# google-research/se3ds

Hardware: AMD Instinct MI355X
Metric: panoramas/sec (G+D train step) at 512x1024 RGB-D (higher is better)
Workload: dtype bf16; 1 GPU; configs/highres 512x1024 full GAN step train_g_d (G+D+hinge+depth+wc losses, clip, Adam, EMA), ResNet-101 gen_dims 128, per-GPU batch 8, d_step_per_g_step 1; per_gpu_batch=8, global_batch=8, parallelism=dp1

## Files before the change

### include/se3ds_hip.h

```cpp
#ifndef SE3DS_HIP_H_
#define SE3DS_HIP_H_

#include <stddef.h>
#include <stdint.h>

#ifdef __cplusplus
extern "C" {
#endif

#define SE3DS_OK 0
#define SE3DS_E_BADSHAPE (-1)
#define SE3DS_E_BADDTYPE (-2)
#define SE3DS_E_WORKSPACE (-3)
#define SE3DS_E_LAUNCH (-4)
#define SE3DS_E_UNSUPPORTED (-5)

#define SE3DS_F32 0
#define SE3DS_I32 1
#define SE3DS_U8 2
#define SE3DS_BF16 3
#define SE3DS_FEAT_BYTE_RANGE 0x100
#define SE3DS_XYZ1_ONES_PRESET 0x200

const char* se3ds_version(void);
// ... 249 lines not shown
int se3ds_pad2d(const void* x, int dtype, int n, int h, int w, int c, int pad, int mode, int wrap_w,
                float value, void* y, void* stream);
int se3ds_head_fwd(const void* x, int dtype, int64_t n, int kind, float* y, void* stream);
int se3ds_head_bwd(const float* dy, const float* y, const void* x, int dtype, int64_t n, int kind,
                   void* dx, void* stream);

int se3ds_sample_sum(const float* a, const float* b, const float* m, int n, int64_t p, int c,
                     int mode, float* out, float* workspace , void* stream);
int se3ds_l1_grad(const float* a, const float* b, const float* m, const float* m2,
                  const float* coef, int n, int64_t p, int c, int mode, float* grad, void* stream);
int se3ds_recip_clamp(const float* sums, int n, float scale, float* out, void* stream);
int se3ds_hinge(const void* logits, int dtype, int64_t half, float cd, float cg, float* sums,
                void* dlog_d, void* dlog_g, void* stream);

int se3ds_multi_sqnorm(const float* grads, const int64_t* chunks, int64_t nchunks,
                       const int64_t* tensor_chunk_start, int ntensors, float* partial,
                       float* sqnorm, void* stream);
int se3ds_multi_clip_by_norm(float* grads, const int64_t* chunks, int64_t nchunks,
                             const float* sqnorm, int ntensors, float clip_norm,
                             float* mean_norm_out, void* stream);
int se3ds_mean_clipped_norm(const float* sqnorm, int ntensors, float clip_norm, float* out,
                            void* stream);
int se3ds_multi_adam_keras(float* params, const float* grads, float* m, float* v, int64_t n,
                           float lr, float beta1, float beta2, float eps, int64_t step,
                           void* stream);
int se3ds_multi_adam_keras_ema(float* params, const float* grads, float* m, float* v, int64_t n,
                               float lr, float beta1, float beta2, float eps, int64_t step,
                               float* ema, float one_minus_decay, void* stream);
int se3ds_multi_clip_adam_keras_ema(float* params, const float* grads, float* m, float* v,
                                    const int64_t* chunks, int64_t nchunks, const float* sqnorm,
                                    float clip_norm, const int64_t* tensor_sn, float lr, float beta1,
                                    float beta2, float eps, int64_t step, float* ema,
                                    float one_minus_decay, void* stream);
int se3ds_multi_ema(float* ema, const float* vars, int64_t n, float one_minus_decay, void* stream);

int se3ds_spectral_table_fields(void);
int se3ds_spectral_part_rows(void);
int se3ds_spectral_vpart_len(void);
int se3ds_spectral_power_iter(const int64_t* table, int nlayers, int training, void* stream);
int se3ds_spectral_bwd_fixup(const int64_t* table, int nlayers, void* stream);
int se3ds_spectral_bwd_dots(const int64_t* table, int nlayers, void* stream);
int se3ds_multi_sqnorm_sn(const float* grads, const int64_t* chunks, int64_t nchunks,
                          const int64_t* tensor_chunk_start, int ntensors, float* partial,
                          float* sqnorm, const int64_t* tensor_sn, int tensor_base, void* stream);
int se3ds_multi_clip_by_norm_sn(float* grads, const int64_t* chunks, int64_t nchunks,
                                const float* sqnorm, int ntensors, float clip_norm,
                                float* mean_norm_out, const int64_t* tensor_sn, void* stream);


int se3ds_input_transform(const uint8_t* image, const uint8_t* proj_image, const uint16_t* depth,
                          const uint16_t* proj_depth, const uint8_t* proj_mask,
                          const uint8_t* blurred_mask, const uint8_t* segmentation,
                          const int32_t* iparams, const float* fparams, int n, int h0, int w0, int h,
                          int w, float* o_image, float* o_proj_image, float* o_proj_mask,
                          float* o_proj_depth, float* o_depth, float* o_blurred, int32_t* o_seg,
                          void* stream);

int se3ds_video_transform(const float* image, const uint8_t* segmentation,
                          const uint8_t* pd_segmentation, const float* depth, const float* pd_depth,
                          const int32_t* hmode, const float* hband, int n, int t, int h0, int w0,
                          int h, int w, float* o_original, float* o_image, uint8_t* o_seg,
                          uint8_t* o_pd_seg, float* o_depth, float* o_pd_depth, void* stream);

int se3ds_png_unfilter(const uint8_t* src, int64_t src_bytes, const int64_t* table,
                       const int64_t* host_table, int n, void* stream);
int se3ds_png_unfilter_fields(void);
int se3ds_png_unfilter_max_row_bytes(void);

int se3ds_png_inflate(const uint8_t* buf, int64_t buf_bytes, uint8_t* workspace,
                      int64_t workspace_bytes, const int64_t* host_table, int n,
                      int32_t* status_dev, void* stream);
int se3ds_png_inflate_fields(void);
int se3ds_png_inflate_ring_bytes(void);

// ... 31 lines not shown
```

### se3ds_amd/csrc/optim.hip

```cpp
#include "common.h"
#include <cmath>

namespace se3ds {
namespace {

constexpr int kB = 256;

__global__ void __launch_bounds__(kB)
chunk_sqsum_kernel(const float* __restrict__ g, const int64_t* __restrict__ chunks,
                   float* __restrict__ partial, const int64_t* __restrict__ tensor_sn) {
  __shared__ float sh[kB / 64];
  const int64_t start = chunks[blockIdx.x * 3 + 1], len = chunks[blockIdx.x * 3 + 2];
  if (tensor_sn && tensor_sn[chunks[blockIdx.x * 3]] != 0) {
    if (threadIdx.x == 0) partial[blockIdx.x] = 0.f;
    return;
  }
  float s = 0.f;
  const float* gp = g + start;
  const int64_t n4 = (((uintptr_t)gp & 15) == 0) ? (len >> 2) : 0;
  float s1 = 0.f, s2 = 0.f, s3 = 0.f;
  for (int64_t i = threadIdx.x; i < n4; i += kB) {
    const float4 v = reinterpret_cast<const float4*>(gp)[i];
    s += v.x * v.x;
    s1 += v.y * v.y;
// ... 187 lines not shown
      const int c = (int)(e - k * C);
      const float vk = sv[k];
      const float4 u4 = *reinterpret_cast<const float4*>(su + c);
      gc[0] = clip_sn(g4.x, inv, coef, vk, u4.x, clip, den);
      gc[1] = clip_sn(g4.y, inv, coef, vk, u4.y, clip, den);
      gc[2] = clip_sn(g4.z, inv, coef, vk, u4.z, clip, den);
      gc[3] = clip_sn(g4.w, inv, coef, vk, u4.w, clip, den);
    }
    adam_elem(gc[0], p4.x, m4.x, v4.x, alpha, b1, b2, eps);
    adam_elem(gc[1], p4.y, m4.y, v4.y, alpha, b1, b2, eps);
    adam_elem(gc[2], p4.z, m4.z, v4.z, alpha, b1, b2, eps);
    adam_elem(gc[3], p4.w, m4.w, v4.w, alpha, b1, b2, eps);
    *reinterpret_cast<float4*>(m + o) = m4;
    *reinterpret_cast<float4*>(v + o) = v4;
    *reinterpret_cast<float4*>(p + o) = p4;
    if (EMA) {
      float4 e4 = *reinterpret_cast<const float4*>(ema + o);
      e4.x = ema_elem(e4.x, p4.x, omd); e4.y = ema_elem(e4.y, p4.y, omd);
      e4.z = ema_elem(e4.z, p4.z, omd); e4.w = ema_elem(e4.w, p4.w, omd);
      *reinterpret_cast<float4*>(ema + o) = e4;
    }
  }
  for (int64_t i = len4 + threadIdx.x; i < len; i += kB) {
    const int64_t o = start + i;
    float pi = p[o], mi = m[o], vi = v[o];
    adam_elem(one(i, g[o]), pi, mi, vi, alpha, b1, b2, eps);
    m[o] = mi;
    v[o] = vi;
    p[o] = pi;
    if (EMA) ema[o] = ema_elem(ema[o], pi, omd);
  }
}

__global__ void __launch_bounds__(kB)
ema_kernel(float* __restrict__ ema, const float* __restrict__ var, int64_t n, float omd) {
  for (int64_t i = (int64_t)blockIdx.x * kB + threadIdx.x; i < n; i += (int64_t)gridDim.x * kB)
    ema[i] = ema[i] - (ema[i] - var[i]) * omd;
}

constexpr int SN_F = 10;
constexpr int SN_KB = 32;
constexpr float SN_EPS = 1e-10f;

__global__ void __launch_bounds__(kB)
sn_v_kernel(const int64_t* __restrict__ tab) {
  const int64_t* L = tab + (int64_t)blockIdx.y * SN_F;
  const float* W = (const float*)L[0];
  const float* u = (const float*)L[1];
  float* v = (float*)L[2];
  float* vpart = (float*)L[6];
  const int64_t K = L[7];
  const int C = (int)L[8];
  __shared__ float sh[kB / 64];
  const int lane = threadIdx.x & 63, wave = threadIdx.x >> 6;
  float sq = 0.f;
  for (int64_t k = (int64_t)blockIdx.x * 4 + wave; k < K; k += (int64_t)SN_RB * 4) {
    float s = 0.f;
    for (int c = lane; c < C; c += 64) s += W[k * C + c] * u[c];
    s = wave_sum(s);
    if (lane == 0) { v[k] = s; sq += s * s; }
  }
  if (lane == 0) sh[wave] = sq;
  __syncthreads();
  if (threadIdx.x == 0) vpart[blockIdx.x] = (sh[0] + sh[1]) + (sh[2] + sh[3]);
}

// ... 139 lines not shown
        const float gv = G[k * C + c];
        dot += gv * W[k * C + c];
        gg += gv * gv;
        row += gv * uhat[c];
      }
    }
    gvu += row * vk;
  }
  dot = wave_sum(dot);
  gg = wave_sum(gg);
  gvu = wave_sum(gvu);
  if (lane == 0) { sh[0][wave] = dot; sh[1][wave] = gg; sh[2][wave] = gvu; }
  __syncthreads();
  if (threadIdx.x < 3) {
    const float* q = sh[threadIdx.x];
    vpart[threadIdx.x * SN_RB + blockIdx.x] = (q[0] + q[1]) + (q[2] + q[3]);
  }
  if (blockIdx.x == 0) {
    __syncthreads();
    float nv = 0.f, nu = 0.f;
    for (int64_t k = threadIdx.x; k < K; k += kB) nv += v[k] * v[k];
    for (int c = threadIdx.x; c < C; c += kB) nu += uhat[c] * uhat[c];
    nv = wave_sum(nv);
    nu = wave_sum(nu);
    if (lane == 0) { sh[0][wave] = nv; sh[1][wave] = nu; }
    __syncthreads();
    if (threadIdx.x < 2) {
      const float* q = sh[threadIdx.x];
      vpart[3 * SN_RB + threadIdx.x] = (q[0] + q[1]) + (q[2] + q[3]);
    }
  }
}

__global__ void __launch_bounds__(kB)
sn_sqnorm_kernel(const int64_t* __restrict__ tensor_sn, int tensor_base, int T,
                 float* __restrict__ sqnorm) {
  for (int t = blockIdx.x * kB + threadIdx.x; t < T; t += gridDim.x * kB) {
    const int64_t* L = (const int64_t*)tensor_sn[tensor_base + t];
    if (L == nullptr) continue;
    const float* sig = (const float*)L[4];
    const float* vpart = (const float*)L[6];
    const float dot = sn_dot_gw(vpart);
    double gg = 0.0, gvu = 0.0;
    for (int i = 0; i < SN_RB; ++i) {
      gg += (double)vpart[SN_RB + i];
      gvu += (double)vpart[2 * SN_RB + i];
    }
    const float inv = sig[1];
    const float coef = inv * inv * dot;
    const double nvu = (double)vpart[3 * SN_RB] * (double)vpart[3 * SN_RB + 1];
    double sq = (double)inv * inv * gg - 2.0 * (double)inv * coef * gvu + (double)coef * coef * nvu;
    sqnorm[t] = sq > 0.0 ? (float)sq : 0.f;
  }
}

}
}

using namespace se3ds;

static float adam_alpha(float lr, float beta1, float beta2, int64_t step) {
  float b1p = (float)pow((double)beta1, (double)step);
  float b2p = (float)pow((double)beta2, (double)step);
  return lr * sqrtf(1.0f - b2p) / (1.0f - b1p);
}

// ... 62 lines not shown

int se3ds_multi_adam_keras_ema(float* params, const float* grads, float* m, float* v, int64_t n,
                               float lr, float beta1, float beta2, float eps, int64_t step,
                               float* ema, float one_minus_decay, void* stream) {
  if (ema == nullptr)
    return se3ds_multi_adam_keras(params, grads, m, v, n, lr, beta1, beta2, eps, step, stream);
  if (n <= 0) return SE3DS_OK;
  float alpha = adam_alpha(lr, beta1, beta2, step);
  hipLaunchKernelGGL(adam_ema_kernel, dim3(grid_for(n, kB)), dim3(kB), 0, as_stream(stream), params,
                     grads, m, v, n, alpha, beta1, beta2, eps, ema, one_minus_decay);
  return check_launch("multi_adam_keras_ema");
}

int se3ds_multi_clip_adam_keras_ema(float* params, const float* grads, float* m, float* v,
                                    const int64_t* chunks, int64_t nchunks, const float* sqnorm,
                                    float clip_norm, const int64_t* tensor_sn, float lr, float beta1,
                                    float beta2, float eps, int64_t step, float* ema,
                                    float one_minus_decay, void* stream) {
  if (nchunks <= 0) return SE3DS_OK;
  if ((((uintptr_t)params | (uintptr_t)grads | (uintptr_t)m | (uintptr_t)v | (uintptr_t)ema) & 15) != 0)
    return SE3DS_E_UNSUPPORTED;
  const float alpha = adam_alpha(lr, beta1, beta2, step);
  if (ema)
    hipLaunchKernelGGL(clip_adam_kernel<true>, dim3((unsigned)nchunks), dim3(kB), 0, as_stream(stream),
                       params, grads, m, v, chunks, sqnorm, clip_norm, tensor_sn, alpha, beta1, beta2,
                       eps, ema, one_minus_decay);
  else
    hipLaunchKernelGGL(clip_adam_kernel<false>, dim3((unsigned)nchunks), dim3(kB), 0, as_stream(stream),
                       params, grads, m, v, chunks, sqnorm, clip_norm, tensor_sn, alpha, beta1, beta2,
                       eps, ema, one_minus_decay);
  return check_launch("multi_clip_adam_keras_ema");
}

int se3ds_multi_ema(float* ema, const float* vars, int64_t n, float one_minus_decay,
                    void* stream) {
  if (n <= 0) return SE3DS_OK;
  hipLaunchKernelGGL(ema_kernel, dim3(grid_for(n, kB)), dim3(kB), 0, as_stream(stream), ema, vars,
                     n, one_minus_decay);
  return check_launch("multi_ema");
}

int se3ds_spectral_power_iter(const int64_t* table, int nlayers, int training, void* stream) {
  if (nlayers <= 0) return SE3DS_OK;
  hipStream_t s = as_stream(stream);
  hipLaunchKernelGGL(sn_v_kernel, dim3(SN_RB, (unsigned)nlayers), dim3(kB), 0, s, table);
  hipLaunchKernelGGL(sn_u_kernel, dim3(SN_KB, (unsigned)nlayers), dim3(kB), 0, s, table);
  hipLaunchKernelGGL(sn_finish_kernel, dim3((unsigned)nlayers), dim3(kB), 0, s, table, training);
  return check_launch("spectral_power_iter");
}

int se3ds_spectral_bwd_fixup(const int64_t* table, int nlayers, void* stream) {
  if (nlayers <= 0) return SE3DS_OK;
  hipStream_t s = as_stream(stream);
  hipLaunchKernelGGL(sn_dot_kernel, dim3(SN_RB, (unsigned)nlayers), dim3(kB), 0, s, table);
  hipLaunchKernelGGL(sn_fix_kernel, dim3(SN_RB, (unsigned)nlayers), dim3(kB), 0, s, table);
  return check_launch("spectral_bwd_fixup");
}

int se3ds_spectral_bwd_dots(const int64_t* table, int nlayers, void* stream) {
  if (nlayers <= 0) return SE3DS_OK;
  hipLaunchKernelGGL(sn_dots_kernel, dim3(SN_RB, (unsigned)nlayers), dim3(kB), 0, as_stream(stream),
                     table);
  return check_launch("spectral_bwd_dots");
}

int se3ds_spectral_table_fields(void) { return SN_F; }
int se3ds_spectral_part_rows(void) { return SN_KB; }
int se3ds_spectral_vpart_len(void) { return 3 * SN_RB + 2; }

}
```

### se3ds_amd/hipops/__init__.py

```python
import ctypes

from se3ds_amd import _lib
from se3ds_amd._lib import c_int, c_i64, c_f, c_p, c_sz

_lib.register({
    'se3ds_weight_prep': (c_int, [c_p, c_i64, c_int, c_int, c_p, c_p, c_p]),
    'se3ds_weight_prep_multi': (c_int, [c_p, c_int, c_i64, c_p]),
    'se3ds_conv2d_fwd': (c_int, [c_p, c_p, c_p, c_int] + [c_int] * 13 + [c_p, c_int, c_p, c_p, c_p,
                                                                      c_p, c_int, c_f, c_p]),
    'se3ds_conv2d_fwd_stats': (c_int, [c_p, c_p, c_p, c_int] + [c_int] * 13 + [c_p, c_int, c_p, c_p,
                                                                            c_p, c_p, c_int, c_f, c_p,
                                                                            c_p]),
    'se3ds_conv2d_fwd_stats_rows': (c_i64, [c_int] * 11),
    'se3ds_conv_transpose2x2_fwd': (c_int, [c_p, c_p, c_p, c_int, c_int, c_int, c_int, c_int, c_int, c_p, c_p]),
    'se3ds_conv2d_dgrad': (c_int, [c_p, c_p, c_p, c_int] + [c_int] * 13 + [c_p, c_p, c_p, c_p,
                                                                        c_int, c_f, c_p]),
    'se3ds_conv2d_dgrad_acc': (c_int, [c_p, c_p, c_p, c_int] + [c_int] * 13 + [c_p, c_p, c_p, c_p,
                                                                        c_int, c_f, c_p, c_p]),
    'se3ds_conv2d_dgrad_bnstats_rows': (c_i64, [c_int] * 10),
    'se3ds_conv2d_dgrad_bnstats': (c_int, [c_p, c_p, c_p, c_int] + [c_int] * 13 +
                                   [c_p, c_p, c_p, c_p, c_p, c_p, c_p, c_int, c_f, c_p, c_p]),
    'se3ds_conv2d_wgrad_workspace_bytes': (c_sz, [c_int] * 7),
    'se3ds_conv2d_wgrad': (c_int, [c_p, c_p, c_p, c_int] + [c_int] * 13 + [c_p, c_int, c_p, c_p, c_int,
                                                                        c_p, c_sz, c_p]),
# ... 28 lines not shown
    'se3ds_norm_bwd_cg_col_rows': (c_int, [c_i64, c_int]),
    'se3ds_norm_bwd_cg': (c_int, [c_p, c_p, c_int, c_i64, c_int, c_p, c_p, c_p, c_f, c_int, c_f, c_p,
                                  c_p, c_p, c_int, c_f, c_p, c_p, c_p, c_p, c_p, c_p, c_p, c_sz, c_p]),
    'se3ds_norm_bwd_apply_rows': (c_int, [c_p, c_p, c_int, c_i64, c_int, c_p, c_p, c_p, c_p, c_f,
                                          c_int, c_f, c_p, c_p, c_p, c_p, c_p, c_p, c_p, c_sz, c_p]),
    'se3ds_affine_bwd': (c_int, [c_p, c_p, c_int, c_int, c_i64, c_int, c_p, c_int, c_f, c_p, c_p,
                                 c_p, c_p]),
    'se3ds_act_bwd': (c_int, [c_p, c_p, c_int, c_i64, c_int, c_f, c_p, c_p]),
    'se3ds_add': (c_int, [c_p, c_p, c_int, c_i64, c_p, c_p]),
    'se3ds_row_scale': (c_int, [c_p, c_int, c_i64, c_int, c_p, c_p, c_p]),
    'se3ds_maxpool2x2_fwd': (c_int, [c_p, c_int, c_int, c_int, c_int, c_int, c_p, c_p]),
    'se3ds_maxpool2x2_bwd': (c_int, [c_p, c_p, c_p, c_int, c_int, c_int, c_int, c_int, c_p, c_p]),
    'se3ds_avgpool3s2_fwd': (c_int, [c_p, c_int, c_int, c_int, c_int, c_int, c_p, c_p]),
    'se3ds_avgpool3s2_bwd': (c_int, [c_p, c_int, c_int, c_int, c_int, c_int, c_p, c_p]),
    'se3ds_upsample2x_fwd': (c_int, [c_p, c_int, c_int, c_int, c_int, c_int, c_p, c_p]),
    'se3ds_upsample2x_bwd': (c_int, [c_p, c_int, c_int, c_int, c_int, c_int, c_p, c_p]),
    'se3ds_copy_channels': (c_int, [c_p, c_int, c_int, c_int, c_p, c_int, c_int, c_int, c_int,
                                    c_i64, c_p]),
    'se3ds_fill': (c_int, [c_p, c_int, c_i64, c_f, c_p]),
    'se3ds_head_fwd': (c_int, [c_p, c_int, c_i64, c_int, c_p, c_p]),
    'se3ds_head_bwd': (c_int, [c_p, c_p, c_p, c_int, c_i64, c_int, c_p, c_p]),
    'se3ds_sample_sum': (c_int, [c_p, c_p, c_p, c_int, c_i64, c_int, c_int, c_p, c_p, c_p]),
    'se3ds_l1_grad': (c_int, [c_p, c_p, c_p, c_p, c_p, c_int, c_i64, c_int, c_int, c_p, c_p]),
    'se3ds_recip_clamp': (c_int, [c_p, c_int, c_f, c_p, c_p]),
    'se3ds_hinge': (c_int, [c_p, c_int, c_i64, c_f, c_f, c_p, c_p, c_p, c_p]),
    'se3ds_multi_sqnorm': (c_int, [c_p, c_p, c_i64, c_p, c_int, c_p, c_p, c_p]),
    'se3ds_multi_clip_by_norm': (c_int, [c_p, c_p, c_i64, c_p, c_int, c_f, c_p, c_p]),
    'se3ds_mean_clipped_norm': (c_int, [c_p, c_int, c_f, c_p, c_p]),
    'se3ds_multi_adam_keras': (c_int, [c_p, c_p, c_p, c_p, c_i64, c_f, c_f, c_f, c_f, c_i64, c_p]),
    'se3ds_multi_adam_keras_ema': (c_int, [c_p, c_p, c_p, c_p, c_i64, c_f, c_f, c_f, c_f, c_i64, c_p,
                                           c_f, c_p]),
    'se3ds_multi_clip_adam_keras_ema': (c_int, [c_p, c_p, c_p, c_p, c_p, c_i64, c_p, c_f, c_p, c_f, c_f,
                                                c_f, c_f, c_i64, c_p, c_f, c_p]),
    'se3ds_multi_ema': (c_int, [c_p, c_p, c_i64, c_f, c_p]),
    'se3ds_spectral_table_fields': (c_int, []),
    'se3ds_spectral_part_rows': (c_int, []),
    'se3ds_spectral_vpart_len': (c_int, []),
    'se3ds_spectral_power_iter': (c_int, [c_p, c_int, c_int, c_p]),
    'se3ds_spectral_bwd_fixup': (c_int, [c_p, c_int, c_p]),
    'se3ds_spectral_bwd_dots': (c_int, [c_p, c_int, c_p]),
    'se3ds_multi_sqnorm_sn': (c_int, [c_p, c_p, c_i64, c_p, c_int, c_p, c_p, c_p, c_int, c_p]),
    'se3ds_multi_clip_by_norm_sn': (c_int, [c_p, c_p, c_i64, c_p, c_int, c_f, c_p, c_p, c_p]),
    'se3ds_quantize': (c_int, [c_p, c_int, c_i64, c_int, c_f, c_f, c_f, c_f, c_f, c_f, c_p, c_int, c_p]),
    'se3ds_pad2d': (c_int, [c_p, c_int, c_int, c_int, c_int, c_int, c_int, c_int, c_int, c_f, c_p,
                            c_p]),
})
```

### se3ds_amd/hipops/nn.py

```python
import math
import threading
from typing import List, Optional

import numpy as np
import os

import torch
import torch.distributed as dist

from se3ds_amd import _lib
from se3ds_amd import hipops

ACT_NONE, ACT_RELU, ACT_LRELU = 0, 1, 2
BN_EPS, BN_MOMENTUM = 1e-3, 0.99
IN_EPS = 1e-3


def _L():
  return _lib.lib()


def _log_collective(kind, numel):
  from se3ds_amd.trainers import dist_utils
  dist_utils.log_collective(kind, numel)


def _all_reduce_sum(t, group, kind):
  from se3ds_amd.trainers import dist_utils
  dist_utils.all_reduce_sum(t, group, kind)


def _chk(rc, what):
# ... 664 lines not shown
    self._copies[dtype] = (version, wt, wn)
    return wt, wn


class OperandGroup:

  def __init__(self, layers: List['ConvLayer'], dtype, device):
    self.dtype = dtype
    self.batched, self.single, rows, tile0 = [], [], [], 0
    for l in layers:
      w = l.kernel
      K, co = w.shape[0] * w.shape[1] * w.shape[2], w.shape[3]
      if dtype == torch.bfloat16 and K % 8 == 0 and co % 4 == 0:
        ent = l._copies.get(dtype)
        if ent is None:
          wt = torch.empty((co, K), dtype=dtype, device=w.device)
          wn = torch.empty((K, co), dtype=dtype, device=w.device)
          l._copies[dtype] = (-1, wt, wn)
        else:
          wt, wn = ent[1], ent[2]
        if (w.data_ptr() | wt.data_ptr()) % 16 == 0 and wn.data_ptr() % 8 == 0:
          rows.append([w.data_ptr(), K, co, wt.data_ptr(), wn.data_ptr(), tile0])
          tile0 += ((K + 63) // 64) * ((co + 63) // 64)
          self.batched.append(l)
          continue
      self.single.append(l)
    self.tiles = tile0
    self.table = torch.tensor(rows, dtype=torch.int64, device=device) if rows else None

  def prep(self, version):
    if self.table is not None:
      _chk(_L().se3ds_weight_prep_multi(self.table.data_ptr(), len(self.batched), self.tiles,
                                        _lib.stream()), 'se3ds_weight_prep_multi')
      for l in self.batched:
        ent = l._copies[self.dtype]
        l._copies[self.dtype] = (version, ent[1], ent[2])
    for l in self.single:
      l.prep(self.dtype, version)


class SpectralGroup:

  def __init__(self, layers: List[ConvLayer], device):
    self.layers = [l for l in layers if l.spectral]
    L = _L()
    nf, pr, vl = (L.se3ds_spectral_table_fields(), L.se3ds_spectral_part_rows(),
                  L.se3ds_spectral_vpart_len())
    rows = []
    for l in self.layers:
      w = l.kernel
      K, co = w.shape[0] * w.shape[1] * w.shape[2], w.shape[3]
      l.sn = dict(v=torch.zeros(K, device=device), uhat=torch.zeros(co, device=device),
                  sig=torch.ones(2, device=device), part=torch.zeros(pr * co, device=device),
                  vpart=torch.zeros(vl, device=device))
      rows.append([w.data_ptr(), l.store[l.name + '/u'].data_ptr(), l.sn['v'].data_ptr(),
                   l.sn['uhat'].data_ptr(), l.sn['sig'].data_ptr(), l.sn['part'].data_ptr(),
                   l.sn['vpart'].data_ptr(), K, co, 0])
      assert len(rows[-1]) == nf
    self._rows = rows
    self.table = torch.tensor(rows, dtype=torch.int64, device=device) if rows else None
    self._eff = [i for i, l in enumerate(self.layers) if l.kind == 'spectral']
    self._eff_table = None

  @property
  def eff_table(self):
    if self._eff_table is None and self._eff:
      rows = []
      for i in self._eff:
        l = self.layers[i]
        r = list(self._rows[i])
        r[9] = l.store.grad_views[l.name + '/kernel'].data_ptr()
        rows.append(r)
      self._eff_table = torch.tensor(rows, dtype=torch.int64, device=self.table.device)
    return self._eff_table

  def power_iteration(self, training):
    if self.table is not None:
      _chk(_L().se3ds_spectral_power_iter(self.table.data_ptr(), self.table.shape[0],
                                          1 if training else 0, _lib.stream()),
           'se3ds_spectral_power_iter')

  def tensor_sn(self, store):
    tab = self.eff_table
    if tab is None:
      return None
    if getattr(self, '_tensor_sn', None) is None:
      nf = tab.shape[1]
      index = {n_: t for t, n_ in enumerate(store.trainable_names)}
      rows = [0] * len(store.trainable_names)
      for j, i in enumerate(self._eff):
        rows[index[self.layers[i].name + '/kernel']] = tab.data_ptr() + 8 * nf * j
      self._tensor_sn = torch.tensor(rows, dtype=torch.int64, device=tab.device)
    return self._tensor_sn

  def backward_fixup(self, prefix=None, dots_only=False):
    tab = self.eff_table
    if tab is None:
      return
    if prefix is not None:
      cache = self.__dict__.setdefault('_seg_tables', {})
      if prefix not in cache:
        pres = prefix if isinstance(prefix, (tuple, list)) else (prefix,)
        rows = [j for j, i in enumerate(self._eff)
                if any(self.layers[i].name.startswith(pre + '/') for pre in pres)]
        cache[prefix] = tab[rows].contiguous() if rows else None
      tab = cache[prefix]
      if tab is None:
        return
    if dots_only:
      _chk(_L().se3ds_spectral_bwd_dots(tab.data_ptr(), tab.shape[0], _lib.stream()),
           'se3ds_spectral_bwd_dots')
      return
    _chk(_L().se3ds_spectral_bwd_fixup(tab.data_ptr(), tab.shape[0], _lib.stream()),
         'se3ds_spectral_bwd_fixup')


_CHECK_MASKS = os.environ.get('SE3DS_CHECK_MASKS') == '1'


def mask_window(ctx, mask, n, h, w, ho, wo, k, stride, pad_t, pad_l, wrap, want_bwd):
  if _CHECK_MASKS and ctx.binary_masks and not bool(((mask == 0) | (mask == 1)).all()):
    raise _lib.Se3dsHipError('a partial-conv mask with values outside {0, 1} reached a binary-mask fast path: '
                             'set gan.binary_masks = False (ctx.binary_masks) for fractional masks')
  ratio = torch.empty((n, ho, wo), dtype=torch.float32, device=ctx.device)
  um = torch.empty_like(ratio)
  ru = torch.empty_like(ratio) if want_bwd else None
  bu = torch.empty_like(ratio) if want_bwd else None
  _chk(_L().se3ds_mask_window(mask.data_ptr(), n, h, w, ho, wo, k, k, stride, pad_t, pad_l,
                              1 if wrap else 0, ratio.data_ptr(), um.data_ptr(), _lib.ptr(ru),
                              _lib.ptr(bu), _lib.stream()), 'se3ds_mask_window')
  return ratio, um, ru, bu


def _colsum(ctx, t2d_ptr, dtype_code, rows, c, row_scale=None, groups=1, out=None):
  sums = torch.empty((groups, 2, c), dtype=torch.float32, device=ctx.device)
  L = _L()
  ws = ctx.ws('norm', L.se3ds_norm_workspace_bytes(groups, c))
  _chk(L.se3ds_norm_stats(t2d_ptr, dtype_code, groups, rows, c, _lib.ptr(row_scale),
                          sums.data_ptr(), _lib.ptr(out), ws.data_ptr(), ws.numel(),
                          _lib.stream()), 'se3ds_norm_stats')
  return sums


_RED_TABLES = {}


def _wgrad(ctx, layer, args, wsz):
# ... 661 lines not shown
```

### se3ds_amd/trainers/gan_manager.py

```python
import abc
import csv
import os
import random
import re
import struct
import zlib
from typing import Optional

import numpy as np
import torch
import torch.distributed as dist

from se3ds_amd import _lib
from se3ds_amd import gin_lite as gin
from se3ds_amd import hipops
from se3ds_amd.trainers import dist_utils
from se3ds_amd.utils import ema


class OneDeviceStrategy:
  num_replicas_in_sync = 1
  group = None

  def __init__(self, device='cuda:0'):
    self.device = torch.device(device)


class DataParallelStrategy:

  def __init__(self, device, group=None):
    self.device = torch.device(device)
    self.group = group
    self.num_replicas_in_sync = dist.get_world_size(group)


class AdamState:

  def __init__(self, model, lr, beta_1, beta_2, epsilon=1e-7):
    self.model = model
    self.lr, self.beta_1, self.beta_2, self.epsilon = lr, beta_1, beta_2, epsilon
    self.m = torch.zeros_like(model.store.theta)
    self.v = torch.zeros_like(model.store.theta)
    self.iterations = 0
    self.chunks, self.tensor_chunk_start = model.store.chunk_tables()
    self._tcs_host = self.tensor_chunk_start.cpu().tolist()
    dev = model.store.theta.device
    self.partial = torch.empty(self.chunks.shape[0], dtype=torch.float32, device=dev)
    self.sqnorm = torch.empty(len(model.store.trainable_names), dtype=torch.float32, device=dev)
# ... 34 lines not shown
    tcs = cache[(t0, t1)]
    _lib.check(L.se3ds_multi_sqnorm_sn(st.grad.data_ptr(), self.chunks.data_ptr() + 24 * c0, c1 - c0,
                                       tcs.data_ptr(), t1 - t0, self.partial.data_ptr(),
                                       self.sqnorm.data_ptr() + 4 * t0, sn, t0, _lib.stream()),
               'se3ds_multi_sqnorm_sn')
    _lib.check(L.se3ds_multi_clip_by_norm_sn(st.grad.data_ptr(), self.chunks.data_ptr() + 24 * c0,
                                             c1 - c0, self.sqnorm.data_ptr(), t1 - t0,
                                             float(clip_norm), None, sn, _lib.stream()),
               'se3ds_multi_clip_by_norm_sn')

  def clip_apply(self, t0, t1, clip_norm=5.0, fused_sn=False, ema_theta=None, one_minus_decay=0.0):
    if self.on_update is not None:
      return False
    st = self.model.store
    L = _lib.lib()
    sn = self._sn_ptr(fused_sn)
    c0, c1 = self._tcs_host[t0], self._tcs_host[t1]
    if c1 <= c0:
      return True
    cache = self.__dict__.setdefault('_seg_tcs', {})
    if (t0, t1) not in cache:
      cache[(t0, t1)] = (self.tensor_chunk_start[t0:t1 + 1] - c0).contiguous()
    tcs = cache[(t0, t1)]
    _lib.check(L.se3ds_multi_sqnorm_sn(st.grad.data_ptr(), self.chunks.data_ptr() + 24 * c0, c1 - c0,
                                       tcs.data_ptr(), t1 - t0, self.partial.data_ptr(),
                                       self.sqnorm.data_ptr() + 4 * t0, sn, t0, _lib.stream()),
               'se3ds_multi_sqnorm_sn')
    _lib.check(L.se3ds_multi_clip_adam_keras_ema(
        st.theta.data_ptr(), st.grad.data_ptr(), self.m.data_ptr(), self.v.data_ptr(),
        self.chunks.data_ptr() + 24 * c0, c1 - c0, self.sqnorm.data_ptr(), float(clip_norm), sn,
        self.lr, self.beta_1, self.beta_2, self.epsilon, self.iterations, _lib.ptr(ema_theta),
        float(one_minus_decay), _lib.stream()), 'se3ds_multi_clip_adam_keras_ema')
    return True

  def mean_clipped_norm(self, clip_norm=5.0):
    _lib.check(_lib.lib().se3ds_mean_clipped_norm(
        self.sqnorm.data_ptr(), len(self.model.store.trainable_names), float(clip_norm),
        self.mean_norm.data_ptr(), _lib.stream()), 'se3ds_mean_clipped_norm')
    return self.mean_norm

  def begin_step(self):
    self.iterations += 1

  def apply_segment(self, e0, e1, ema_theta=None, one_minus_decay=0.0):
    st = self.model.store
    if e1 <= e0:
      return
    if self.on_update is not None:
      self.on_update(e0, e1)
    _lib.check(_lib.lib().se3ds_multi_adam_keras_ema(
        st.theta.data_ptr() + 4 * e0, st.grad.data_ptr() + 4 * e0, self.m.data_ptr() + 4 * e0,
        self.v.data_ptr() + 4 * e0, e1 - e0, self.lr, self.beta_1, self.beta_2, self.epsilon,
        self.iterations, (ema_theta.data_ptr() + 4 * e0) if ema_theta is not None else None,
        float(one_minus_decay), _lib.stream()), 'se3ds_multi_adam_keras_ema')

  def end_step(self):
    self.model.store.version += 1

  def apply_gradients(self, group=None, world=1, ema_theta=None, one_minus_decay=0.0):
    st = self.model.store
    if world > 1:
      dist_utils.allreduce_arena_sum(st.grad, group)
    if self.on_update is not None:
      self.on_update(0, st.theta.numel())
    self.iterations += 1
    _lib.check(_lib.lib().se3ds_multi_adam_keras_ema(
# ... 361 lines not shown
```

### se3ds_amd/trainers/se3ds_trainer.py

```python
import os
from typing import Dict

import torch

from se3ds_amd import _lib
from se3ds_amd import gin_lite as gin
from se3ds_amd.hipops import nn
from se3ds_amd.hipops.nn import Var
from se3ds_amd.models import image_models
from se3ds_amd.trainers import dist_utils
from se3ds_amd.trainers import gan_manager
from se3ds_amd.trainers.gan_manager import Mean

FUSED_SN_CLIP = True
GRAD_CLIP_NORM = 5.0
SEGMENT_OPTIMIZER = os.environ.get('SE3DS_SEGMENT_OPTIMIZER', '1') != '0'
FUSED_CLIP_ADAM = os.environ.get('SE3DS_FUSED_CLIP_ADAM', '1') != '0'
DEFER_WGRAD_REDUCE = os.environ.get('SE3DS_DEFER_WGRAD_REDUCE', '1') != '0'


def _L():
  return _lib.lib()


@gin.configurable(denylist=['strategy', 'model_dir'])
class GAN(gan_manager.GANManager):

  def __init__(self, lambda_gan, lambda_kld, lambda_wc, lambda_depth, *args,
               dis_use_pred_depth=True, mask_blurred=False, **kwargs):
    super().__init__(*args, **kwargs)
    self.lambda_gan = lambda_gan
    self.lambda_kld = lambda_kld
    self.lambda_wc = lambda_wc
    self.lambda_depth = lambda_depth
    self.dis_use_pred_depth = dis_use_pred_depth
    self.mask_blurred = mask_blurred

  def _create_metrics(self):
    names = ['gen/gen_loss', 'dis/disc_loss', 'dis/grad_norm', 'gen/gen_feat_loss',
             'gen/gen_gan_loss', 'gen/depth_loss', 'gen/seg_loss', 'gen/depth_seg_loss',
             'gen/depth_seg_consistency', 'gen/kld_loss', 'gen/kld_nan', 'gen/wc_loss',
             'gen/grad_norm']
    self.metrics = {n: Mean(n.split('/')[-1]) for n in names}

  def _prep_inputs(self, inputs):
    inputs = dict(inputs)
    for k in ('image', 'proj_image', 'proj_depth', 'proj_mask', 'depth', 'blurred_mask'):
      t = inputs[k]
      _lib.require_cuda(t)
      inputs[k] = t.to(torch.float32).contiguous()
    if not self.mask_blurred:
# ... 186 lines not shown
    gx = x_all.grad
    x_all.grad = None
    del tape_d
    g_rgb = nn.slice_channels(gx[:n], 0, 3, torch.float32)
    _lib.check(L.se3ds_add(d_rgb.data_ptr(), g_rgb.data_ptr(), _lib.F32, d_rgb.numel(),
                           d_rgb.data_ptr(), _lib.stream()), 'se3ds_add')
    if self.dis_use_pred_depth:
      g_dep = nn.slice_channels(gx[:n], 3, 1, torch.float32)
      _lib.check(L.se3ds_add(d_depth.data_ptr(), g_dep.data_ptr(), _lib.F32, d_depth.numel(),
                             d_depth.data_ptr(), _lib.stream()), 'se3ds_add')
    ctx_g.param_grads = True
    push_rgb(d_rgb)
    push_depth(d_depth)
    ema_theta, ema_omd = self.ema_fused_args()
    if sync is None and SEGMENT_OPTIMIZER and nn.conv_profiler() is None:
      segs = self._segments()
      opt = self._optimizer_stream(dev)
      main = torch.cuda.current_stream(dev)
      ev = torch.cuda.Event()
      ev.record()
      with torch.cuda.stream(opt):
        opt.wait_event(ev)
        self._update_all(self.d_optimizer, False, None, 0.0)
        d_norm = self.d_optimizer.mean_clipped_norm(GRAD_CLIP_NORM).clone()
      self.g_optimizer.begin_step()
      def segment_done(name):
        if name not in segs:
          return
        t0, t1, e0, e1 = segs[name]
        done = torch.cuda.Event()
        done.record()
        with torch.cuda.stream(opt):
          opt.wait_event(done)
          nn.flush_wgrad_reduces(ctx_g)
          G.spectral.backward_fixup(prefix=G.SEGMENTS[name], dots_only=FUSED_SN_CLIP)
          if not (FUSED_CLIP_ADAM and self.g_optimizer.clip_apply(
              t0, t1, GRAD_CLIP_NORM, FUSED_SN_CLIP, ema_theta, ema_omd)):
            self.g_optimizer.clip_segment(t0, t1, GRAD_CLIP_NORM, fused_sn=FUSED_SN_CLIP)
            self.g_optimizer.apply_segment(e0, e1, ema_theta, ema_omd)
          self._operand_group(G, name, ctx_g.dtype).prep(G.store.version + 1)
      ctx_g.on_segment = segment_done
      if DEFER_WGRAD_REDUCE:
        ctx_g.wgrad_defer = []
      ctx_g.backward()
      ctx_g.on_segment = None
      ctx_g.wgrad_defer = None
      with torch.cuda.stream(opt):
        opt.wait_stream(main)
        self._operand_group(D, None, ctx_d.dtype).prep(D.store.version)
      main.wait_stream(opt)
      self.g_optimizer.end_step()
      g_norm = self.g_optimizer.mean_clipped_norm(GRAD_CLIP_NORM).clone()
    elif sync is None:
      if DEFER_WGRAD_REDUCE:
        ctx_g.wgrad_defer = []
      ctx_g.backward()
      ctx_g.wgrad_defer = None
      G.spectral.backward_fixup(dots_only=FUSED_SN_CLIP)
      self._update_all(self.g_optimizer, FUSED_SN_CLIP, ema_theta, ema_omd)
      g_norm = self.g_optimizer.mean_clipped_norm(GRAD_CLIP_NORM).clone()
      self._update_all(self.d_optimizer, False, None, 0.0)
      d_norm = self.d_optimizer.mean_clipped_norm(GRAD_CLIP_NORM).clone()
      self._operand_group(G, None, ctx_g.dtype).prep(G.store.version)
      self._operand_group(D, None, ctx_d.dtype).prep(D.store.version)
    else:
      opt = self._optimizer_stream(dev)
      main = torch.cuda.current_stream(dev)
      opt.wait_stream(main)
      def segment_done(name):
        if name not in self._g_segments:
          return
        t0, t1, e0, e1 = self._g_segments[name]
        done = torch.cuda.Event()
# ... 91 lines not shown
```

Baseline: 42.45 panoramas/sec.

## Fuse clip+Adam+EMA with bf16 weight prep per generator segment

```diff
diff --git a/include/se3ds_hip.h b/include/se3ds_hip.h
--- a/include/se3ds_hip.h
+++ b/include/se3ds_hip.h
@@ -305,6 +305,11 @@
                                     float clip_norm, const int64_t* tensor_sn, float lr, float beta1,
                                     float beta2, float eps, int64_t step, float* ema,
                                     float one_minus_decay, void* stream);
+int se3ds_multi_clip_adam_keras_ema_prep(const int64_t* table, int nlayers, int64_t total_tiles,
+                                         const float* sqnorm, float clip_norm, float lr, float beta1,
+                                         float beta2, float eps, int64_t step, float one_minus_decay,
+                                         void* stream);
+int se3ds_clip_adam_prep_table_fields(void);
 int se3ds_multi_ema(float* ema, const float* vars, int64_t n, float one_minus_decay, void* stream);
 
 int se3ds_spectral_table_fields(void);
@@ -313,6 +318,8 @@
 int se3ds_spectral_power_iter(const int64_t* table, int nlayers, int training, void* stream);
 int se3ds_spectral_bwd_fixup(const int64_t* table, int nlayers, void* stream);
 int se3ds_spectral_bwd_dots(const int64_t* table, int nlayers, void* stream);
+int se3ds_spectral_bwd_dots_reduce(const int64_t* table, int nlayers, const int64_t* src_table,
+                                   void* stream);
 int se3ds_multi_sqnorm_sn(const float* grads, const int64_t* chunks, int64_t nchunks,
                           const int64_t* tensor_chunk_start, int ntensors, float* partial,
                           float* sqnorm, const int64_t* tensor_sn, int tensor_base, void* stream);
diff --git a/se3ds_amd/csrc/optim.hip b/se3ds_amd/csrc/optim.hip
--- a/se3ds_amd/csrc/optim.hip
+++ b/se3ds_amd/csrc/optim.hip
@@ -243,6 +243,111 @@
   }
 }
 
+constexpr int AP_F = 12;
+__global__ void __launch_bounds__(kB)
+clip_adam_prep_kernel(const int64_t* __restrict__ table, int nlayers, const float* __restrict__ sqnorm,
+                      float clip, float alpha, float b1, float b2, float eps, float omd) {
+  __shared__ float tile[64][65];
+  const int64_t blk = blockIdx.x;
+  int lo = 0, hi = nlayers - 1;
+  while (lo < hi) {
+    const int mid = (lo + hi + 1) >> 1;
+    if (table[(int64_t)mid * AP_F + 11] <= blk) lo = mid; else hi = mid - 1;
+  }
+  const int64_t* R = table + (int64_t)lo * AP_F;
+  float* __restrict__ p = (float*)R[0];
+  const float* __restrict__ g = (const float*)R[1];
+  float* __restrict__ m = (float*)R[2];
+  float* __restrict__ v = (float*)R[3];
+  float* __restrict__ ema = (float*)R[4];
+  uint16_t* __restrict__ wt = (uint16_t*)R[5];
+  uint16_t* __restrict__ wn = (uint16_t*)R[6];
+  const int64_t K = R[7];
+  const int Cout = (int)R[8];
+  const float sq = sqnorm[R[9]];
+  const float norm = sq > 0.f ? sqrtf(sq) : sq;
+  const float den = fmaxf(norm, clip);
+  const int64_t* L = (const int64_t*)R[10];
+  const float* sv = nullptr;
+  const float* su = nullptr;
+  float inv = 0.f, coef = 0.f;
+  if (L != nullptr) {
+    sv = (const float*)L[2];
+    su = (const float*)L[3];
+    const float* sig = (const float*)L[4];
+    const float* vpart = (const float*)L[6];
+    const float dot = sn_dot_gw(vpart);
+    inv = sig[1];
+    coef = inv * inv * dot;
+  }
+  const int64_t local = blk - R[11];
+  const int64_t tiles_k = (K + 63) / 64;
+  const int64_t k0 = (local % tiles_k) * 64;
+  const int c0 = (int)(local / tiles_k) * 64;
+  const int tid = threadIdx.x;
+  {
+    const int cq = (tid & 15) * 4, r0 = tid >> 4;
+#pragma unroll
+    for (int i = 0; i < 4; ++i) {
+      const int r = r0 + 16 * i;
+      const int64_t k = k0 + r;
+      const int c = c0 + cq;
+      float4 p4 = make_float4(0.f, 0.f, 0.f, 0.f);
+      if (k < K && c < Cout) {
+        const int64_t o = k * Cout + c;
+        const float4 g4 = *reinterpret_cast<const float4*>(g + o);
+        p4 = *reinterpret_cast<const float4*>(p + o);
+        float4 m4 = *reinterpret_cast<const float4*>(m + o);
+        float4 v4 = *reinterpret_cast<const float4*>(v + o);
+        float gc[4];
+        if (L == nullptr) {
+          gc[0] = clip_plain(g4.x, clip, den); gc[1] = clip_plain(g4.y, clip, den);
+          gc[2] = clip_plain(g4.z, clip, den); gc[3] = clip_plain(g4.w, clip, den);
+        } else {
+          const float vk = sv[k];
+          const float4 u4 = *reinterpret_cast<const float4*>(su + c);
+          gc[0] = clip_sn(g4.x, inv, coef, vk, u4.x, clip, den);
+          gc[1] = clip_sn(g4.y, inv, coef, vk, u4.y, clip, den);
+          gc[2] = clip_sn(g4.z, inv, coef, vk, u4.z, clip, den);
+          gc[3] = clip_sn(g4.w, inv, coef, vk, u4.w, clip, den);
+        }
+        adam_elem(gc[0], p4.x, m4.x, v4.x, alpha, b1, b2, eps);
+        adam_elem(gc[1], p4.y, m4.y, v4.y, alpha, b1, b2, eps);
+        adam_elem(gc[2], p4.z, m4.z, v4.z, alpha, b1, b2, eps);
+        adam_elem(gc[3], p4.w, m4.w, v4.w, alpha, b1, b2, eps);
+        *reinterpret_cast<float4*>(m + o) = m4;
+        *reinterpret_cast<float4*>(v + o) = v4;
+        *reinterpret_cast<float4*>(p + o) = p4;
+        if (ema != nullptr) {
+          float4 e4 = *reinterpret_cast<const float4*>(ema + o);
+          e4.x = ema_elem(e4.x, p4.x, omd); e4.y = ema_elem(e4.y, p4.y, omd);
+          e4.z = ema_elem(e4.z, p4.z, omd); e4.w = ema_elem(e4.w, p4.w, omd);
+          *reinterpret_cast<float4*>(ema + o) = e4;
+        }
+        uint16_t ob[4] = {f32_to_bf16(p4.x), f32_to_bf16(p4.y), f32_to_bf16(p4.z), f32_to_bf16(p4.w)};
+        *reinterpret_cast<uint2*>(wn + o) = *reinterpret_cast<const uint2*>(ob);
+      }
+      tile[r][cq] = p4.x; tile[r][cq + 1] = p4.y; tile[r][cq + 2] = p4.z; tile[r][cq + 3] = p4.w;
+    }
+  }
+  __syncthreads();
+  {
+    const int kq = (tid & 7) * 8, cr0 = tid >> 3;
+#pragma unroll
+    for (int j = 0; j < 2; ++j) {
+      const int cr = cr0 + 32 * j;
+      const int c = c0 + cr;
+      const int64_t k = k0 + kq;
+      if (c < Cout && k < K) {
+        uint16_t ob[8];
+#pragma unroll
+        for (int e = 0; e < 8; ++e) ob[e] = f32_to_bf16(tile[kq + e][cr]);
+        *reinterpret_cast<uint4*>(wt + (int64_t)c * K + k) = *reinterpret_cast<const uint4*>(ob);
+      }
+    }
+  }
+}
+
 __global__ void __launch_bounds__(kB)
 ema_kernel(float* __restrict__ ema, const float* __restrict__ var, int64_t n, float omd) {
   for (int64_t i = (int64_t)blockIdx.x * kB + threadIdx.x; i < n; i += (int64_t)gridDim.x * kB)
@@ -448,6 +553,111 @@
   }
 }
 
+__device__ __forceinline__ float4 slab_sum4(const float4* __restrict__ P, int splits, int64_t n4,
+                                            int64_t i) {
+  float4 s0 = make_float4(0.f, 0.f, 0.f, 0.f), s1 = s0, s2 = s0, s3 = s0;
+  auto add = [](float4& a, const float4& b) { a.x += b.x; a.y += b.y; a.z += b.z; a.w += b.w; };
+  int k = 0;
+  for (; k + 3 < splits; k += 4) {
+    const float4 a = P[(int64_t)k * n4 + i], b = P[(int64_t)(k + 1) * n4 + i];
+    const float4 c = P[(int64_t)(k + 2) * n4 + i], d = P[(int64_t)(k + 3) * n4 + i];
+    add(s0, a); add(s1, b); add(s2, c); add(s3, d);
+  }
+  for (; k < splits; ++k) add(s0, P[(int64_t)k * n4 + i]);
+  return make_float4(((s0.x + s1.x) + (s2.x + s3.x)) * 1.0f, ((s0.y + s1.y) + (s2.y + s3.y)) * 1.0f,
+                     ((s0.z + s1.z) + (s2.z + s3.z)) * 1.0f, ((s0.w + s1.w) + (s2.w + s3.w)) * 1.0f);
+}
+
+__global__ void __launch_bounds__(kB)
+sn_dots_reduce_kernel(const int64_t* __restrict__ tab, const int64_t* __restrict__ src) {
+  const int64_t* L = tab + (int64_t)blockIdx.y * SN_F;
+  const float* W = (const float*)L[0];
+  const float* v = (const float*)L[2];
+  const float* uhat = (const float*)L[3];
+  float* vpart = (float*)L[6];
+  float* G = (float*)L[9];
+  const int64_t K = L[7];
+  const int C = (int)L[8];
+  const float* P = (const float*)src[(int64_t)blockIdx.y * 2];
+  const int splits = (int)src[(int64_t)blockIdx.y * 2 + 1];
+  __shared__ float sh[3][kB / 64];
+  const int lane = threadIdx.x & 63, wave = threadIdx.x >> 6;
+  float dot = 0.f, gg = 0.f, gvu = 0.f;
+  const bool vec = (C & 3) == 0 &&
+                   ((((uintptr_t)G | (uintptr_t)W | (uintptr_t)uhat | (uintptr_t)P) & 15) == 0);
+  const int64_t n4 = (K * C) >> 2;
+  for (int64_t k = (int64_t)blockIdx.x * 4 + wave; k < K; k += (int64_t)SN_RB * 4) {
+    const float vk = v[k];
+    float row = 0.f;
+    if (vec) {
+      float4* G4 = reinterpret_cast<float4*>(G + k * C);
+      const float4* W4 = reinterpret_cast<const float4*>(W + k * C);
+      const float4* U4 = reinterpret_cast<const float4*>(uhat);
+      const float4* P4 = reinterpret_cast<const float4*>(P);
+      const int64_t i0 = (k * C) >> 2;
+      const int nq = C >> 2;
+      for (int c = lane; c < nq; c += 64) {
+        float4 gv;
+        if (splits > 0) {
+          gv = slab_sum4(P4, splits, n4, i0 + c);
+          G4[c] = gv;
+        } else {
+          gv = G4[c];
+        }
+        const float4 wv = W4[c], uv = U4[c];
+        dot += (gv.x * wv.x + gv.y * wv.y) + (gv.z * wv.z + gv.w * wv.w);
+        gg += (gv.x * gv.x + gv.y * gv.y) + (gv.z * gv.z + gv.w * gv.w);
+        row += (gv.x * uv.x + gv.y * uv.y) + (gv.z * uv.z + gv.w * uv.w);
+      }
+    } else {
+      for (int c = lane; c < C; c += 64) {
+        float gv;
+        if (splits > 0) {
+          const int64_t n = K * C, e = k * C + c;
+          float s0 = 0.f, s1 = 0.f, s2 = 0.f, s3 = 0.f;
+          int j = 0;
+          for (; j + 3 < splits; j += 4) {
+            s0 += P[(int64_t)j * n + e]; s1 += P[(int64_t)(j + 1) * n + e];
+            s2 += P[(int64_t)(j + 2) * n + e]; s3 += P[(int64_t)(j + 3) * n + e];
+          }
+          for (; j < splits; ++j) s0 += P[(int64_t)j * n + e];
+          gv = ((s0 + s1) + (s2 + s3)) * 1.0f;
+          G[k * C + c] = gv;
+        } else {
+          gv = G[k * C + c];
+        }
+        dot += gv * W[k * C + c];
+        gg += gv * gv;
+        row += gv * uhat[c];
+      }
+    }
+    gvu += row * vk;
+  }
+  dot = wave_sum(dot);
+  gg = wave_sum(gg);
+  gvu = wave_sum(gvu);
+  if (lane == 0) { sh[0][wave] = dot; sh[1][wave] = gg; sh[2][wave] = gvu; }
+  __syncthreads();
+  if (threadIdx.x < 3) {
+    const float* q = sh[threadIdx.x];
+    vpart[threadIdx.x * SN_RB + blockIdx.x] = (q[0] + q[1]) + (q[2] + q[3]);
+  }
+  if (blockIdx.x == 0) {
+    __syncthreads();
+    float nv = 0.f, nu = 0.f;
+    for (int64_t k = threadIdx.x; k < K; k += kB) nv += v[k] * v[k];
+    for (int c = threadIdx.x; c < C; c += kB) nu += uhat[c] * uhat[c];
+    nv = wave_sum(nv);
+    nu = wave_sum(nu);
+    if (lane == 0) { sh[0][wave] = nv; sh[1][wave] = nu; }
+    __syncthreads();
+    if (threadIdx.x < 2) {
+      const float* q = sh[threadIdx.x];
+      vpart[3 * SN_RB + threadIdx.x] = (q[0] + q[1]) + (q[2] + q[3]);
+    }
+  }
+}
+
 __global__ void __launch_bounds__(kB)
 sn_sqnorm_kernel(const int64_t* __restrict__ tensor_sn, int tensor_base, int T,
                  float* __restrict__ sqnorm) {
@@ -576,6 +786,18 @@
   return check_launch("multi_clip_adam_keras_ema");
 }
 
+int se3ds_multi_clip_adam_keras_ema_prep(const int64_t* table, int nlayers, int64_t total_tiles,
+                                         const float* sqnorm, float clip_norm, float lr, float beta1,
+                                         float beta2, float eps, int64_t step, float one_minus_decay,
+                                         void* stream) {
+  if (nlayers <= 0 || total_tiles <= 0) return SE3DS_OK;
+  const float alpha = adam_alpha(lr, beta1, beta2, step);
+  hipLaunchKernelGGL(clip_adam_prep_kernel, dim3((unsigned)total_tiles), dim3(kB), 0, as_stream(stream),
+                     table, nlayers, sqnorm, clip_norm, alpha, beta1, beta2, eps, one_minus_decay);
+  return check_launch("multi_clip_adam_keras_ema_prep");
+}
+int se3ds_clip_adam_prep_table_fields(void) { return AP_F; }
+
 int se3ds_multi_ema(float* ema, const float* vars, int64_t n, float one_minus_decay,
                     void* stream) {
   if (n <= 0) return SE3DS_OK;
@@ -608,6 +830,14 @@
   return check_launch("spectral_bwd_dots");
 }
 
+int se3ds_spectral_bwd_dots_reduce(const int64_t* table, int nlayers, const int64_t* src_table,
+                                   void* stream) {
+  if (nlayers <= 0) return SE3DS_OK;
+  hipLaunchKernelGGL(sn_dots_reduce_kernel, dim3(SN_RB, (unsigned)nlayers), dim3(kB), 0,
+                     as_stream(stream), table, src_table);
+  return check_launch("spectral_bwd_dots_reduce");
+}
+
 int se3ds_spectral_table_fields(void) { return SN_F; }
 int se3ds_spectral_part_rows(void) { return SN_KB; }
 int se3ds_spectral_vpart_len(void) { return 3 * SN_RB + 2; }
diff --git a/se3ds_amd/hipops/__init__.py b/se3ds_amd/hipops/__init__.py
--- a/se3ds_amd/hipops/__init__.py
+++ b/se3ds_amd/hipops/__init__.py
@@ -84,6 +84,9 @@
                                            c_f, c_p]),
     'se3ds_multi_clip_adam_keras_ema': (c_int, [c_p, c_p, c_p, c_p, c_p, c_i64, c_p, c_f, c_p, c_f, c_f,
                                                 c_f, c_f, c_i64, c_p, c_f, c_p]),
+    'se3ds_multi_clip_adam_keras_ema_prep': (c_int, [c_p, c_int, c_i64, c_p, c_f, c_f, c_f, c_f, c_f, c_i64,
+                                                     c_f, c_p]),
+    'se3ds_clip_adam_prep_table_fields': (c_int, []),
     'se3ds_multi_ema': (c_int, [c_p, c_p, c_i64, c_f, c_p]),
     'se3ds_spectral_table_fields': (c_int, []),
     'se3ds_spectral_part_rows': (c_int, []),
@@ -91,6 +94,7 @@
     'se3ds_spectral_power_iter': (c_int, [c_p, c_int, c_int, c_p]),
     'se3ds_spectral_bwd_fixup': (c_int, [c_p, c_int, c_p]),
     'se3ds_spectral_bwd_dots': (c_int, [c_p, c_int, c_p]),
+    'se3ds_spectral_bwd_dots_reduce': (c_int, [c_p, c_int, c_p, c_p]),
     'se3ds_multi_sqnorm_sn': (c_int, [c_p, c_p, c_i64, c_p, c_int, c_p, c_p, c_p, c_int, c_p]),
     'se3ds_multi_clip_by_norm_sn': (c_int, [c_p, c_p, c_i64, c_p, c_int, c_f, c_p, c_p, c_p]),
     'se3ds_quantize': (c_int, [c_p, c_int, c_i64, c_int, c_f, c_f, c_f, c_f, c_f, c_f, c_p, c_int, c_p]),
diff --git a/se3ds_amd/hipops/nn.py b/se3ds_amd/hipops/nn.py
--- a/se3ds_amd/hipops/nn.py
+++ b/se3ds_amd/hipops/nn.py
@@ -1,3 +1,4 @@
+import collections
 import math
 import threading
 from typing import List, Optional
@@ -728,9 +729,12 @@
     if self.table is not None:
       _chk(_L().se3ds_weight_prep_multi(self.table.data_ptr(), len(self.batched), self.tiles,
                                         _lib.stream()), 'se3ds_weight_prep_multi')
-      for l in self.batched:
-        ent = l._copies[self.dtype]
-        l._copies[self.dtype] = (version, ent[1], ent[2])
+    self.stamp(version)
+
+  def stamp(self, version):
+    for l in self.batched:
+      ent = l._copies[self.dtype]
+      l._copies[self.dtype] = (version, ent[1], ent[2])
     for l in self.single:
       l.prep(self.dtype, version)
 
@@ -767,6 +771,7 @@
         r = list(self._rows[i])
         r[9] = l.store.grad_views[l.name + '/kernel'].data_ptr()
         rows.append(r)
+      self._eff_rows = rows
       self._eff_table = torch.tensor(rows, dtype=torch.int64, device=self.table.device)
     return self._eff_table
 
@@ -809,6 +814,69 @@
       return
     _chk(_L().se3ds_spectral_bwd_fixup(tab.data_ptr(), tab.shape[0], _lib.stream()),
          'se3ds_spectral_bwd_fixup')
+
+
+  def backward_dots_reduce(self, ctx, prefix):
+    rows = ctx.wgrad_defer or []
+    if ctx.wgrad_defer is not None:
+      ctx.wgrad_defer = []
+    tab = self.eff_table
+    if tab is None:
+      if rows:
+        _reduce_rows(ctx, rows)
+      return
+    key = (prefix, tuple(rows))
+    cache = self.__dict__.setdefault('_fused_tables', {})
+    ent = cache.get(key)
+    if ent is None:
+      pres = prefix if isinstance(prefix, (tuple, list)) else (prefix,)
+      sn_rows = [self._eff_rows[j] for j, i in enumerate(self._eff)
+                 if any(self.layers[i].name.startswith(pre + '/') for pre in pres)]
+      fused, src, old, rest = plan_dots_reduce(sn_rows, rows)
+      dev = tab.device
+      mk = lambda r: torch.tensor(r, dtype=torch.int64, device=dev) if r else None
+      ent = (mk(fused), mk(src), mk(old), rest)
+      if len(cache) >= 256:
+        cache.clear()
+      cache[key] = ent
+    fused, src, old, rest = ent
+    if rest:
+      _reduce_rows(ctx, rest)
+    if fused is not None:
+      fused_calls['dots_reduce'] += 1
+      _chk(_L().se3ds_spectral_bwd_dots_reduce(fused.data_ptr(), fused.shape[0], src.data_ptr(),
+                                               _lib.stream()), 'se3ds_spectral_bwd_dots_reduce')
+    if old is not None:
+      _chk(_L().se3ds_spectral_bwd_dots(old.data_ptr(), old.shape[0], _lib.stream()),
+           'se3ds_spectral_bwd_dots')
+
+
+fused_calls = collections.Counter()
+
+
+def plan_dots_reduce(sn_rows, red_rows):
+  by_dst = {}
+  for r in red_rows:
+    by_dst.setdefault(r[3], []).append(r)
+  fused, src, old, taken = [], [], [], set()
+  for row in sn_rows:
+    w, uhat, K, co, g = row[0], row[3], row[7], row[8], row[9]
+    mine = by_dst.get(g, [])
+    vec = co % 4 == 0 and (w | uhat | g) % 16 == 0
+    if vec and not mine:
+      fused.append(list(row))
+      src.append([0, 0])
+    elif (vec and len(mine) == 1 and mine[0][1] > 0 and mine[0][0] % 16 == 0 and
+          mine[0][2] * 4 == K * co):
+      fused.append(list(row))
+      src.append([mine[0][0], mine[0][1]])
+      taken.add(tuple(mine[0]))
+    else:
+      old.append(list(row))
+  if not taken:
+    return [], [], [list(r) for r in sn_rows], list(red_rows)
+  rest = [r for r in red_rows if tuple(r) not in taken]
+  return fused, src, old, rest
 
 
 _CHECK_MASKS = os.environ.get('SE3DS_CHECK_MASKS') == '1'
diff --git a/se3ds_amd/trainers/gan_manager.py b/se3ds_amd/trainers/gan_manager.py
--- a/se3ds_amd/trainers/gan_manager.py
+++ b/se3ds_amd/trainers/gan_manager.py
@@ -14,6 +14,7 @@
 from se3ds_amd import _lib
 from se3ds_amd import gin_lite as gin
 from se3ds_amd import hipops
+from se3ds_amd.hipops import nn
 from se3ds_amd.trainers import dist_utils
 from se3ds_amd.utils import ema
 
@@ -114,6 +115,80 @@
         self.lr, self.beta_1, self.beta_2, self.epsilon, self.iterations, _lib.ptr(ema_theta),
         float(one_minus_decay), _lib.stream()), 'se3ds_multi_clip_adam_keras_ema')
     return True
+
+  def clip_apply_prep(self, t0, t1, group, version, clip_norm=5.0, fused_sn=False, ema_theta=None,
+                      one_minus_decay=0.0):
+    if self.on_update is not None or group.table is None:
+      return False
+    st = self.model.store
+    L = _lib.lib()
+    sn = self._sn_ptr(fused_sn)
+    c0, c1 = self._tcs_host[t0], self._tcs_host[t1]
+    if c1 <= c0:
+      return False
+    ema_ptr = ema_theta.data_ptr() if ema_theta is not None else 0
+    cache = self.__dict__.setdefault('_seg_prep', {})
+    key = (t0, t1, id(group), ema_ptr, sn or 0)
+    if key not in cache:
+      cache[key] = self._prep_tables(t0, t1, group, ema_ptr, sn)
+    ent = cache[key]
+    if ent is None:
+      return False
+    table, nlayers, tiles, rest, _group = ent
+    tcs_cache = self.__dict__.setdefault('_seg_tcs', {})
+    if (t0, t1) not in tcs_cache:
+      tcs_cache[(t0, t1)] = (self.tensor_chunk_start[t0:t1 + 1] - c0).contiguous()
+    tcs = tcs_cache[(t0, t1)]
+    _lib.check(L.se3ds_multi_sqnorm_sn(st.grad.data_ptr(), self.chunks.data_ptr() + 24 * c0, c1 - c0,
+                                       tcs.data_ptr(), t1 - t0, self.partial.data_ptr(),
+                                       self.sqnorm.data_ptr() + 4 * t0, sn, t0, _lib.stream()),
+               'se3ds_multi_sqnorm_sn')
+    nn.fused_calls['adam_prep'] += 1
+    _lib.check(L.se3ds_multi_clip_adam_keras_ema_prep(
+        table.data_ptr(), nlayers, tiles, self.sqnorm.data_ptr(), float(clip_norm), self.lr,
+        self.beta_1, self.beta_2, self.epsilon, self.iterations, float(one_minus_decay),
+        _lib.stream()), 'se3ds_multi_clip_adam_keras_ema_prep')
+    if rest is not None:
+      _lib.check(L.se3ds_multi_clip_adam_keras_ema(
+          st.theta.data_ptr(), st.grad.data_ptr(), self.m.data_ptr(), self.v.data_ptr(),
+          rest.data_ptr(), rest.shape[0], self.sqnorm.data_ptr(), float(clip_norm), sn,
+          self.lr, self.beta_1, self.beta_2, self.epsilon, self.iterations, _lib.ptr(ema_theta),
+          float(one_minus_decay), _lib.stream()), 'se3ds_multi_clip_adam_keras_ema')
+    group.stamp(version)
+    return True
+
+  def _prep_tables(self, t0, t1, group, ema_ptr, sn):
+    st = self.model.store
+    L = _lib.lib()
+    bases = (st.theta.data_ptr(), st.grad.data_ptr(), self.m.data_ptr(), self.v.data_ptr())
+    if any(b % 16 for b in bases + (ema_ptr,)):
+      return None
+    index = {n_: t for t, n_ in enumerate(st.trainable_names)}
+    sn_host = None
+    if sn is not None:
+      sn_host = self.model.spectral.tensor_sn(st).cpu().tolist()
+    rows, tiled, tile0 = [], set(), 0
+    for l in group.batched:
+      name = l.name + '/kernel'
+      t = index.get(name)
+      if l.store is not st or t is None or not t0 <= t < t1:
+        return None
+      o, n_, shape = st._off_tr[name]
+      K, co = shape[0] * shape[1] * shape[2], shape[3]
+      _, wt, wn = l._copies[group.dtype]
+      assert K * co == n_ and K % 8 == 0 and co % 4 == 0 and st.theta.data_ptr() + 4 * o == l.kernel.data_ptr()
+      rows.append([b + 4 * o for b in bases] + [ema_ptr + 4 * o if ema_ptr else 0, wt.data_ptr(),
+                                                wn.data_ptr(), K, co, t, sn_host[t] if sn_host else 0,
+                                                tile0])
+      assert len(rows[-1]) == L.se3ds_clip_adam_prep_table_fields()
+      tile0 += ((K + 63) // 64) * ((co + 63) // 64)
+      tiled.add(t)
+    c0, c1 = self._tcs_host[t0], self._tcs_host[t1]
+    chunks = self.chunks[c0:c1].cpu().tolist()
+    rest = [c for c in chunks if c[0] not in tiled]
+    dev = st.theta.device
+    rest_t = torch.tensor(rest, dtype=torch.int64, device=dev).reshape(-1, 3).contiguous() if rest else None
+    return torch.tensor(rows, dtype=torch.int64, device=dev), len(rows), tile0, rest_t, group
 
   def mean_clipped_norm(self, clip_norm=5.0):
     _lib.check(_lib.lib().se3ds_mean_clipped_norm(
diff --git a/se3ds_amd/trainers/se3ds_trainer.py b/se3ds_amd/trainers/se3ds_trainer.py
--- a/se3ds_amd/trainers/se3ds_trainer.py
+++ b/se3ds_amd/trainers/se3ds_trainer.py
@@ -17,6 +17,8 @@
 SEGMENT_OPTIMIZER = os.environ.get('SE3DS_SEGMENT_OPTIMIZER', '1') != '0'
 FUSED_CLIP_ADAM = os.environ.get('SE3DS_FUSED_CLIP_ADAM', '1') != '0'
 DEFER_WGRAD_REDUCE = os.environ.get('SE3DS_DEFER_WGRAD_REDUCE', '1') != '0'
+FUSED_REDUCE_DOTS = False
+FUSED_ADAM_PREP = True
 
 
 def _L():
@@ -269,13 +271,20 @@
         done.record()
         with torch.cuda.stream(opt):
           opt.wait_event(done)
-          nn.flush_wgrad_reduces(ctx_g)
-          G.spectral.backward_fixup(prefix=G.SEGMENTS[name], dots_only=FUSED_SN_CLIP)
+          if FUSED_REDUCE_DOTS and FUSED_SN_CLIP:
+            G.spectral.backward_dots_reduce(ctx_g, G.SEGMENTS[name])
+          else:
+            nn.flush_wgrad_reduces(ctx_g)
+            G.spectral.backward_fixup(prefix=G.SEGMENTS[name], dots_only=FUSED_SN_CLIP)
+          group = self._operand_group(G, name, ctx_g.dtype)
+          if FUSED_ADAM_PREP and FUSED_CLIP_ADAM and self.g_optimizer.clip_apply_prep(
+              t0, t1, group, G.store.version + 1, GRAD_CLIP_NORM, FUSED_SN_CLIP, ema_theta, ema_omd):
+            return
           if not (FUSED_CLIP_ADAM and self.g_optimizer.clip_apply(
               t0, t1, GRAD_CLIP_NORM, FUSED_SN_CLIP, ema_theta, ema_omd)):
             self.g_optimizer.clip_segment(t0, t1, GRAD_CLIP_NORM, fused_sn=FUSED_SN_CLIP)
             self.g_optimizer.apply_segment(e0, e1, ema_theta, ema_omd)
-          self._operand_group(G, name, ctx_g.dtype).prep(G.store.version + 1)
+          group.prep(G.store.version + 1)
       ctx_g.on_segment = segment_done
       if DEFER_WGRAD_REDUCE:
         ctx_g.wgrad_defer = []
```

After: 42.43 panoramas/sec. No clear change (-0.0%).
